# haoheliu/ssr_eval

Measured on AMD Instinct MI355X. Metric: utterance-pairs/sec (LSD+SSIM, 48kHz, n_fft=2048), higher is better.
Workload: dtype f64

## Files before the change

### ssr_eval_amd/csrc/ssr_metrics.h

```cpp
#pragma once
#include "ssr_stft.h"

#define SSR_SSIM_NT 64
#define SSR_SSIM_MAXCPT 6
#define SSR_SSIM_WIN 7

SSR_HD constexpr int ssr_ssim_strip_out(int cpt) { return SSR_SSIM_NT * cpt; }
SSR_HD int ssr_ssim_pick_cpt(int n_bins) {
  const int outs = n_bins - (SSR_SSIM_WIN - 1);
  if (outs <= SSR_SSIM_NT * 4) {
    int c = (outs + SSR_SSIM_NT - 1) / SSR_SSIM_NT;
    return c < 1 ? 1 : c;
  }
  int best = 4, best_waste = 1 << 30;
  for (int c = 4; c <= SSR_SSIM_MAXCPT; ++c) {
    const int w = SSR_SSIM_NT * c;
    const int waste = ((outs + w - 1) / w) * w - outs;
    if (waste < best_waste) { best_waste = waste; best = c; }
  }
  return best;
}

struct SsrSsimParams {
  const float* x;
  const float* y;
  const int64_t* frame_off;
  const int32_t* n_rows;
  int F;
  int rows_per_tile, n_row_tiles, n_strips;
  double* part;
  int pitch;
  int vi_n;
  int64_t x_plane;
};
SSR_DEV int ssr_ssim_pitch(const SsrSsimParams& p) { return p.pitch ? p.pitch : p.F; }

template <int CPT> struct SsrSsimRegs {
  double cs[CPT + 1][4];
  double s;
  float px[2][4][CPT + 1];
  float ring[SSR_SSIM_WIN][CPT + 1];
  double pxy[CPT], pb[CPT];
  float den[CPT];
};

template <int CPT> SSR_DEV int ssr_ssim_slot(int c) { return (CPT % 2 == 0) ? c + c / CPT : c; }
template <int CPT> SSR_DEV int ssr_ssim_slot_of(int tid, int d) { return (CPT % 2 == 0) ? (CPT + 1) * tid + (d + d / CPT) : CPT * tid + d; }

template <int CPT, bool CONTIG = false> struct SsrSsimLds {
  static constexpr int PW = SSR_SSIM_NT * CPT + 8 + ((CPT % 2 == 0) ? (SSR_SSIM_NT * CPT + 8) / CPT + 1 : 0);
  static constexpr int NQ = CONTIG ? 1 : 4;
  static constexpr int RW = SSR_SSIM_NT * CPT + 8;
  static constexpr size_t ring_bytes() { return CONTIG ? sizeof(float) * SSR_SSIM_WIN * RW : 0; }
  static constexpr size_t bytes() { return ring_bytes() + sizeof(double) * (NQ * PW + SSR_SSIM_NT + 16 + 8); }
  float* yring; double* col; double* sc0; double* sc1; double* res;
  SSR_MEMBER explicit SsrSsimLds(char* base) {
    yring = reinterpret_cast<float*>(base);
    col = reinterpret_cast<double*>(base + ring_bytes());
    sc0 = col + NQ * PW;
    sc1 = sc0 + SSR_SSIM_NT;
    res = sc1 + 16;
  }
};

SSR_DEV void ssr_ld4(const float* p, float* o) {
#ifdef SSR_HOST_EMU
  memcpy(o, p, 16);
#else
  typedef float f4 __attribute__((ext_vector_type(4)));
  const f4 v = *reinterpret_cast<const f4*>(p);
  o[0] = v.x; o[1] = v.y; o[2] = v.z; o[3] = v.w;
#endif
}
SSR_DEV void ssr_st4(float* p, const float* v) {
#ifdef SSR_HOST_EMU
  memcpy(p, v, 16);
#else
  typedef float f4 __attribute__((ext_vector_type(4)));
  *reinterpret_cast<f4*>(p) = f4{v[0], v[1], v[2], v[3]};
#endif
}

struct SsrImage {
#ifdef SSR_HOST_EMU
  const float* base;
  SSR_MEMBER SsrImage(const float* p, int64_t) : base(p) {}
// ... 94 lines not shown
    R.cs[i][1] = (R.cs[i][1] + b) - dd;
    R.cs[i][2] = fma(-dd, dd, fma(-c, c, fma(b, b, fma(a, a, R.cs[i][2]))));
    R.cs[i][3] = fma(-c, dd, fma(a, b, R.cs[i][3]));
    R.ring[SLOT][i] = R.px[SET][0][i];
    ssr_touch(R.ring[SLOT][i]);
  }
}

struct SsrSsimK {
  static constexpr double n = 49.0;
  static constexpr float cov = (float)(49.0 / 48.0);
  static constexpr float C1n = (float)((0.01 * 2.0) * (0.01 * 2.0) * 49.0 * 49.0), C2n = (float)((0.03 * 2.0) * (0.03 * 2.0) * 49.0 * 49.0);
};
SSR_DEV void ssr_ssim_stage1(double sx, double sy, double& pxy, double& pp) { pxy = sx * sy; pp = fma(sx, sx, sy * sy); }
SSR_DEV float ssr_ssim_stage2f(double pp, double sq) {
  const double t2 = fma(SsrSsimK::n, sq, -pp);
  const float b1 = (float)pp + SsrSsimK::C1n;
  const float b2 = fmaf(SsrSsimK::cov, (float)t2, SsrSsimK::C2n);
  return b1 * b2;
}
SSR_DEV float ssr_ssim_stage3f(double pxy, double sxy, float b12) {
  const double t1 = fma(SsrSsimK::n, sxy, -pxy);
  const float a1 = fmaf(2.0f, (float)pxy, SsrSsimK::C1n);
  const float a2 = fmaf(2.0f * SsrSsimK::cov, (float)t1, SsrSsimK::C2n);
#ifndef SSR_HOST_EMU
  return (a1 * a2) * __builtin_amdgcn_rcpf(b12);
#else
  return (a1 * a2) / b12;
#endif
}
SSR_DEV double ssr_ssim_value(double sx, double sy, double sq, double sxy) {
  double pxy, pp;
  ssr_ssim_stage1(sx, sy, pxy, pp);
  return (double)ssr_ssim_stage3f(pxy, sxy, ssr_ssim_stage2f(pp, sq));
}

#ifndef SSR_HOST_EMU
#define SSR_SSIM_ST(arr, idx, val) (*(volatile __attribute__((address_space(3))) double*)(&(arr)[idx]) = (val))
#define SSR_SSIM_LD(arr, idx) (*(const volatile __attribute__((address_space(3))) double*)(&(arr)[idx]))
#else
#define SSR_SSIM_ST(arr, idx, val) ((arr)[idx] = (val))
#define SSR_SSIM_LD(arr, idx) ((arr)[idx])
#endif
template <int CPT, bool CONTIG, typename BLK>
SSR_BODY void ssr_ssim_body(const SsrSsimParams& p, BLK& blk, int tile, int item, char* lds_base) {
  constexpr int NT = SSR_SSIM_NT, PW = SsrSsimLds<CPT, CONTIG>::PW, VC = CPT + 1, W = SSR_SSIM_WIN;
  using Regs = SsrSsimRegs<CPT>;
  using Lds = SsrSsimLds<CPT, CONTIG>;
  Lds L(lds_base);
  const int row_tile = tile / p.n_strips, strip = tile % p.n_strips;
  const int item_v = item;
  const float* xbase = p.x;
  if (p.vi_n > 0) { xbase += (int64_t)(item / p.vi_n) * p.x_plane; item = item % p.vi_n; }
  const int T = p.n_rows[item];
  const int out_rows = T - (W - 1);
  const int r0 = row_tile * p.rows_per_tile;
  const int r1 = (r0 + p.rows_per_tile < out_rows) ? r0 + p.rows_per_tile : out_rows;
  const int c_in0 = strip * ssr_ssim_strip_out(CPT);
  const int ncol_in = (p.F - c_in0 < NT * CPT + (W - 1)) ? p.F - c_in0 : NT * CPT + (W - 1);
  const int ncol_out = ncol_in - (W - 1);
  double* part = p.part + (int64_t)item_v * p.n_row_tiles * p.n_strips + tile;
  const int pitch = ssr_ssim_pitch(p);
  const SsrImage x(xbase + p.frame_off[item] * pitch, (int64_t)T * pitch);
  const SsrImage y(p.y + p.frame_off[item] * pitch, (int64_t)T * pitch);

  SSR_REGS(Regs, regs, blk);
  if (r0 >= r1 || ncol_out <= 0) {
    SSR_PHASE(blk, regs, if (tid == 0) *part = 0.0);
    return;
  }
  const int n_steps = (W - 1) + (r1 - r0);
#define SSR_SSIM_STEP(s_, SET, SLOT)                                                                                         \
  SSR_PHASE(blk, regs, {                                                                                                    \
    ssr_ssim_row_apply<CPT, false, SET, SLOT>(R, tid, (s_) >= W, ncol_in);                                                   \
    ssr_ssim_row_load<CPT, false, SET>(p, R, tid, x, y, ssr_ssim_row_ahead(r0 + (s_) + 2, T),                               \
                                       ((s_) + 2 >= W) ? r0 + (s_) + 2 - W : -1, c_in0, ncol_in);                           \
    if ((s_) >= W - 1) {                                                                                                    \
      for (int i = 0; i < VC; ++i) {                                                                                        \
        const int c = ssr_ssim_col<CPT, false>(tid, i);                                                                     \
        if (c < ncol_in)                                                                                                    \
          for (int q = 0; q < 4; ++q) L.col[q * PW + ssr_ssim_slot<CPT>(c)] = R.cs[i][q];                                    \
      }                                                                                                                     \
    }                                                                                                                       \
  });                                                                                                                       \
  if ((s_) >= W - 1) {                                                                                                      \
    SSR_PHASE(blk, regs, {                                                                                                  \
      const int j0 = tid * CPT;                                                                                             \
      if (j0 < ncol_out) {                                                                                                  \
        double w[4][CPT];                                      \
        for (int q = 0; q < 4; ++q) {                                                                                       \
          double v[CPT + W - 1];                                                                                            \
          for (int d = 0; d < CPT + W - 1; ++d) {                                                                           \
            int c = j0 + d;                                                                                                 \
            if (c >= ncol_in) c = ncol_in - 1;                                \
            v[d] = L.col[q * PW + ssr_ssim_slot<CPT>(c)];                                                                   \
          }                                                                                                                 \
          double sw = v[0];                                                                                                 \
          for (int d = 1; d < W; ++d) sw += v[d];                                                                           \
          w[q][0] = sw;                                                                                                     \
          for (int i = 1; i < CPT; ++i) {                                                                                   \
            sw += v[i + W - 1] - v[i - 1];                                                                                  \
            w[q][i] = sw;                                                                                                   \
          }                                                                                                                 \
        }                                                                                                                   \
        for (int i = 0; i < CPT; ++i)                                                                                       \
          if (j0 + i < ncol_out) R.s += ssr_ssim_value(w[0][i], w[1][i], w[2][i], w[3][i]);                                  \
      }                                                                                                                     \
// ... 109 lines not shown
  }
};

template <typename BLK>
SSR_BODY void ssr_specred_body(const SsrSpecRedParams& p, BLK& blk, int chunk, int item, char* lds_base) {
  constexpr int NT = SsrSpecRedLds::NT;
  SsrSpecRedLds L(lds_base);
  const int T = p.n_rows[item];
  const int t0 = chunk * p.rows_per_chunk;
  const int t1 = (t0 + p.rows_per_chunk < T) ? t0 + p.rows_per_chunk : T;
  const float* x = p.x + p.frame_off[item] * p.F;
  const float* y = p.y + p.frame_off[item] * p.F;
  double* part = p.part + ((int64_t)item * p.n_chunks + chunk) * SSR_NPART;
  const bool want_lsd = p.metric_mask & SSR_M_LSD;
  SSR_REGS(SsrSpecRedRegs, regs, blk);
  SSR_PHASE(blk, regs, for (int q = 0; q < 7; ++q) R.acc[q] = 0.0; R.lsd_sum = 0.0);
  for (int t = t0; t < t1; ++t) {
    SSR_PHASE(blk, regs, {
      R.acc[0] = 0.0;
      for (int k = tid; k < p.F; k += NT)
        ssr_accumulate_metrics(x[(int64_t)t * p.F + k], y[(int64_t)t * p.F + k], p.metric_mask, R.acc);
      L.sc0[tid] = R.acc[0];
    });
    if (want_lsd) {
      SSR_PHASE(blk, regs, if (tid < 16) {
        double s = 0.0;
        for (int i = tid; i < NT; i += 16) s += L.sc0[i];
        L.sc1[tid] = s;
      });
      SSR_PHASE(blk, regs, if (tid == 0) {
        double s = 0.0;
        for (int i = 0; i < 16; ++i) s += L.sc1[i];
        R.lsd_sum += sqrt(s / (double)p.F);
      });
    }
  }
#define SSR_GET_ACC(q) R.acc[(q) + 1]
  SSR_BLOCK_SUM(blk, regs, NT, 6, L.sc0, L.sc1, L.res, SSR_GET_ACC);
#undef SSR_GET_ACC
  SSR_PHASE(blk, regs, if (tid == 0) {
    part[0] = R.lsd_sum;
    for (int q = 0; q < 6; ++q) part[1 + q] = L.res[q];
    part[7] = 0.0;
  });
}

struct SsrFinalizeParams {
  const double* part; int n_chunks;
  const double* ssim_part; int n_tiles;
  const int32_t* n_rows;
  int F, metric_mask, n_items;
  double* out;
  int vi_n, out_keys, out_key0;
};

SSR_DEV double ssr_sispec_from_sums(double sdd, double stt, double sdt) {
  const double EPS = 1e-12;
  const double den = stt + EPS;
  const double alpha = (stt + sdt) / den;
  const double beta = (EPS - sdt) / den;
  const double tt = alpha * alpha * stt;
  double nn = sdd + 2.0 * beta * sdt + beta * beta * stt;
  if (nn < 0.0) nn = 0.0;
  return 10.0 * log10(tt / (nn + EPS) + EPS);
}

SSR_DEV void ssr_finalize_item(const SsrFinalizeParams& p, int item) {
  const double nan_ = NAN;
  const int real = p.vi_n > 0 ? item % p.vi_n : item;
  double* o = p.vi_n > 0 ? p.out + ((int64_t)real * p.out_keys + p.out_key0 + item / p.vi_n) * 4 : p.out + (int64_t)item * 4;
  const int T = p.n_rows[real];
  o[0] = o[1] = o[2] = o[3] = nan_;
  if (p.part) {
    double s[SSR_NPART];
    for (int q = 0; q < SSR_NPART; ++q) s[q] = 0.0;
    for (int c = 0; c < p.n_chunks; ++c)
      for (int q = 0; q < SSR_NPART; ++q) s[q] += p.part[((int64_t)item * p.n_chunks + c) * SSR_NPART + q];
    if (p.metric_mask & SSR_M_LSD) o[0] = s[0] / (double)T;
    if (p.metric_mask & SSR_M_LOG_SISPEC) o[1] = ssr_sispec_from_sums(s[4], s[5], s[6]);
    if (p.metric_mask & SSR_M_SISPEC) o[2] = ssr_sispec_from_sums(s[1], s[2], s[3]);
  }
  if (p.ssim_part && (p.metric_mask & SSR_M_SSIM)) {
    double s = 0.0;
    for (int c = 0; c < p.n_tiles; ++c) s += p.ssim_part[(int64_t)item * p.n_tiles + c];
    o[3] = (T >= SSR_SSIM_WIN && p.F >= SSR_SSIM_WIN) ? s / ((double)(T - 6) * (double)(p.F - 6)) : nan_;
  }
}
```

### ssr_eval_amd/csrc/ssr_specred_wave.h

```cpp
#pragma once
#include "ssr_stft.h"

struct SsrSpecWaveParams {
  const float* x;
  const float* y;
  const int64_t* frame_off;
  const int32_t* n_rows;
  int F, pitch, metric_mask, rows_per_chunk, n_chunks, vi_n;
  int64_t x_plane;
  double* part;
};

struct SsrSpecTgt2 { f2 t, tt, lt; };

__device__ __forceinline__ SsrSpecTgt2 ssr_spec_tgt2(float t0, float t1) {
  const f2 t = f2_make(t0, t1);
  return {t, t * t, ssr_log10f_fast2(t + f2_splat(1e-12f))};
}
__device__ __forceinline__ void ssr_spec_tgt_sums2(const SsrSpecTgt2& y, double* tsum) {
  const double t0 = (double)y.t.x, l0 = (double)y.lt.x, t1 = (double)y.t.y, l1 = (double)y.lt.y;
  tsum[0] += t0 * t0; tsum[1] += l0 * l0;
  tsum[0] += t1 * t1; tsum[1] += l1 * l1;
}
__device__ __forceinline__ void ssr_spec_est2(float e0, float e1, const SsrSpecTgt2& y, double* acc) {
  const f2 EPS2 = f2_splat(1e-12f);
  const f2 e = f2_make(e0, e1);
  const f2 ee = e + EPS2;
  const f2 d = ssr_log10f_fast2(ssr_divf_fast2(y.tt, ee * ee) + EPS2);
  const f2 dd = d * d;
  const f2 le = ssr_log10f_fast2(ee);
  {
    acc[0] += (double)dd.x;
    const double td = (double)y.t.x, d0 = (double)e.x - td;
    acc[1] += d0 * d0; acc[3] += d0 * td;
    const double ld = (double)y.lt.x, l0 = (double)le.x - ld;
    acc[4] += l0 * l0; acc[6] += l0 * ld;
  }
  {
    acc[0] += (double)dd.y;
    const double td = (double)y.t.y, d0 = (double)e.y - td;
    acc[1] += d0 * d0; acc[3] += d0 * td;
    const double ld = (double)y.lt.y, l0 = (double)le.y - ld;
    acc[4] += l0 * l0; acc[6] += l0 * ld;
  }
}

template <int KG>
__device__ __forceinline__ void ssr_specred_wave_body(const SsrSpecWaveParams& p, int chunk, int group_v) {
  const int lane = (int)threadIdx.x;
  const int key0 = (group_v / p.vi_n) * KG, item = group_v % p.vi_n;
  const int T = p.n_rows[item];
  const int t0 = chunk * p.rows_per_chunk;
  const int t1 = (t0 + p.rows_per_chunk < T) ? t0 + p.rows_per_chunk : T;
  const float* x = p.x + (int64_t)key0 * p.x_plane + p.frame_off[item] * (int64_t)p.pitch;
  const float* y = p.y + p.frame_off[item] * (int64_t)p.pitch;
  const int mask = p.metric_mask;
  const bool want_lsd = mask & SSR_M_LSD;
  constexpr int FULL = SSR_M_LSD | SSR_M_SISPEC | SSR_M_LOG_SISPEC;
  const bool fast = (mask & FULL) == FULL;
  double acc[KG][7];
  double lsd_sum[KG];
  double tsum[2] = {0.0, 0.0};
#pragma unroll
  for (int g = 0; g < KG; ++g) {
    lsd_sum[g] = 0.0;
#pragma unroll
    for (int q = 0; q < 7; ++q) acc[g][q] = 0.0;
  }
  const int nq = (p.F + 3) / 4;
  const int nfull = p.F / 4;
  for (int t = t0; t < t1; ++t) {
    const float4* yr = reinterpret_cast<const float4*>(y + (int64_t)t * p.pitch);
#pragma unroll
    for (int g = 0; g < KG; ++g) acc[g][0] = 0.0;
    if (fast) {
      for (int q = lane; q < nfull; q += 64) {
        const float4 yv = yr[q];
        float4 xv[KG];
#pragma unroll
        for (int g = 0; g < KG; ++g) xv[g] = reinterpret_cast<const float4*>(x + (int64_t)g * p.x_plane + (int64_t)t * p.pitch)[q];
        const SsrSpecTgt2 y01 = ssr_spec_tgt2(yv.x, yv.y), y23 = ssr_spec_tgt2(yv.z, yv.w);
        ssr_spec_tgt_sums2(y01, tsum);
        ssr_spec_tgt_sums2(y23, tsum);
#pragma unroll
        for (int g = 0; g < KG; ++g) {
          ssr_spec_est2(xv[g].x, xv[g].y, y01, acc[g]);
          ssr_spec_est2(xv[g].z, xv[g].w, y23, acc[g]);
        }
      }
      if (nfull < nq && lane == nfull % 64) {
        const float4 yv = yr[nfull];
        const int k = 4 * nfull;
        double a7[7];
#pragma unroll
        for (int g = 0; g < KG; ++g) {
          const float4 xv = reinterpret_cast<const float4*>(x + (int64_t)g * p.x_plane + (int64_t)t * p.pitch)[nfull];
          a7[0] = acc[g][0]; a7[1] = acc[g][1]; a7[2] = tsum[0]; a7[3] = acc[g][3]; a7[4] = acc[g][4]; a7[5] = tsum[1]; a7[6] = acc[g][6];
          ssr_accumulate_metrics<true>(xv.x, yv.x, mask, a7);
          if (k + 1 < p.F) ssr_accumulate_metrics<true>(xv.y, yv.y, mask, a7);
          if (k + 2 < p.F) ssr_accumulate_metrics<true>(xv.z, yv.z, mask, a7);
          acc[g][0] = a7[0]; acc[g][1] = a7[1]; acc[g][3] = a7[3]; acc[g][4] = a7[4]; acc[g][6] = a7[6];
          if (g == KG - 1) { tsum[0] = a7[2]; tsum[1] = a7[5]; }
        }
      }
// ... 38 lines not shown
```

### ssr_eval_amd/csrc/ssr_stft.h

```cpp
#pragma once
#include "ssr_fft.h"
#define SSR_UIDX(...) ((unsigned)(__VA_ARGS__))

enum { SSR_MODE_PAIR = 0, SSR_MODE_SINGLE = 1 };

SSR_HD constexpr int ssr_stft_ppt(int logn, bool bluestein) { return logn >= 13 ? 16 : 8; }
enum { SSR_OUT_NONE = 0, SSR_OUT_MAG = 1, SSR_OUT_COMPLEX = 2 };
enum { SSR_M_LSD = 1, SSR_M_LOG_SISPEC = 2, SSR_M_SISPEC = 4, SSR_M_SSIM = 8 };

#define SSR_NPART 8

template <typename T> struct SsrStftParams {
  const float* a;
  const double* a64;
  const double* b64;
  const float* b;
  const int64_t* a_off;
  const int64_t* b_off;
  const int32_t* len;
  const int64_t* frame_off;
  int mode, out_kind, metric_mask;
  int n_fft, hop, n_bins;
  int units_per_chunk;
  int n_chunks;
  int interleave;
  const T* window;
  const cx<T>* tw;
  const cx<T>* wchirp;
  const cx<T>* bfilt;
  const cx<T>* chirp;
  float* out_a;
  float* out_b;
  int out_pitch;
  double* part;
};

enum { SSR_IN_F32 = 0, SSR_IN_EST64 = 1, SSR_IN_BOTH64 = 3, SSR_IN_EST64X2 = 7 };
template <bool F64> struct SsrSample { typedef float type; };
template <> struct SsrSample<true> { typedef double type; };

template <typename T, bool SUMS = false, int PPT = 8> struct SsrStftRegs {
  cx<T> v[PPT];
  double sums[SUMS ? 6 : 1];
  cx<T> twp[3 * (PPT >= 8 ? PPT / 8 : 1)];
};

template <typename T, bool SUMS, int PPT, typename SA, typename SB> struct SsrStftRegsPf : SsrStftRegs<T, SUMS, PPT> {
  SA pa[PPT];
  SB pb[PPT];
  T pw[PPT / 2];
};
template <bool BLUESTEIN, typename T, bool SUMS, int PPT, typename SA, typename SB> struct SsrStftPickRegs {
  typedef SsrStftRegsPf<T, SUMS, PPT, SA, SB> type;
};
template <typename T, bool SUMS, int PPT, typename SA, typename SB> struct SsrStftPickRegs<true, T, SUMS, PPT, SA, SB> {
  typedef SsrStftRegs<T, SUMS, PPT> type;
};


SSR_DEV int ssr_num_frames_dev(int n, int n_fft, int hop) { return 1 + (n + 2 * (n_fft / 2) - n_fft) / hop; }

template <typename T> struct SsrBinOut { float ar, ai, br, bi; };

template <typename T> SSR_DEV SsrBinOut<T> ssr_separate(cx<T> zk, cx<T> zn) {
  SsrBinOut<T> o;
  o.ar = (float)(zk.x + zn.x);
  o.ai = (float)(zk.y - zn.y);
  o.br = (float)(zk.y + zn.y);
  o.bi = (float)(zn.x - zk.x);
  return o;
}

SSR_DEV float ssr_cabsf(float re, float im) { return hypotf(re, im); }

SSR_DEV float ssr_cabsf_fast(float re, float im) {
#ifdef SSR_HOST_EMU
  return sqrtf(fmaf(re, re, im * im));
#else
  return __builtin_amdgcn_sqrtf(__builtin_fmaf(re, re, im * im));
#endif
}

SSR_DEV float ssr_divf_fast(float a, float b) {
#ifdef SSR_HOST_EMU
  return a / b;
#else
  const float r = __builtin_amdgcn_rcpf(b);
  const float q = a * r;
  return __builtin_fmaf(__builtin_fmaf(-q, b, a), r, q);
#endif
}
SSR_DEV float ssr_log10f_fast(float x) {
#ifdef SSR_HOST_EMU
  return log10f(x);
#else
  const float y = __builtin_amdgcn_logf(x);
  const float c = 0x1.344134p-2f, cc = 0x1.09f79ep-26f;
  const float r = y * c;
  return r + __builtin_fmaf(y, cc, __builtin_fmaf(y, c, -r));
#endif
}

SSR_DEV f2 ssr_cabsf_fast2(f2 re, f2 im) {
  const f2 s = f2_fma(re, re, im * im);
#ifdef SSR_HOST_EMU
  return f2_make(sqrtf(s.x), sqrtf(s.y));
#else
  return f2_make(__builtin_amdgcn_sqrtf(s.x), __builtin_amdgcn_sqrtf(s.y));
#endif
}
SSR_DEV f2 ssr_divf_fast2(f2 a, f2 b) {
#ifdef SSR_HOST_EMU
  return f2_make(a.x / b.x, a.y / b.y);
// ... 509 lines not shown
```

### ssr_eval_amd/csrc/tu_metrics.hip

```cpp
#include "ssr_host.h"
#include "ssr_metrics.h"
#include "ssr_pair_transform.h"

template <int CPT, bool CONTIG>
__global__ __launch_bounds__(SSR_SSIM_NT, 1) void k_ssim(SsrSsimParams p) {
  extern __shared__ __attribute__((aligned(16))) char smem[];
  SsrBlk blk{(int)threadIdx.x};
  const int tiles = p.n_row_tiles * p.n_strips;
  ssr_ssim_body<CPT, CONTIG>(p, blk, blockIdx.x % tiles, blockIdx.x / tiles, smem);
}


__global__ __launch_bounds__(256) void k_specred(SsrSpecRedParams p) {
  extern __shared__ __attribute__((aligned(16))) char smem[];
  SsrBlk blk{(int)threadIdx.x};
  ssr_specred_body(p, blk, blockIdx.x % p.n_chunks, blockIdx.x / p.n_chunks, smem);
}

__global__ __launch_bounds__(64) void k_finalize(SsrFinalizeParams p) {
  const int item = blockIdx.x * 64 + threadIdx.x;
  if (item < p.n_items) ssr_finalize_item(p, item);
}

struct SsimGeom { int rows_per_tile, n_row_tiles, n_strips, cpt; };
static SsimGeom ssim_geom(int max_rows, int n_bins, int n_items, bool aligned_rows) {
  SsimGeom g;
  const int out_rows = max_rows - 6 > 1 ? max_rows - 6 : 1;
  int64_t r = ((int64_t)out_rows * n_items + ssr_target_wgs() - 1) / ssr_target_wgs();
  if (r < 8) r = 8;
  if (r > 128) r = 128;
  if (r > out_rows) r = out_rows;
  g.rows_per_tile = (int)r;
  g.n_row_tiles = ssr_ceil_div(out_rows, g.rows_per_tile);
  g.cpt = ssr_ssim_pick_cpt(n_bins);
  if (aligned_rows && g.cpt != 4) {
    const int outs = n_bins - (SSR_SSIM_WIN - 1);
    if (outs > 0) {
      const int strips4 = ssr_ceil_div(outs, ssr_ssim_strip_out(4)), strips_c = ssr_ceil_div(outs, ssr_ssim_strip_out(g.cpt));
      if (strips4 * 5 * 68 < strips_c * (g.cpt + 1) * 100) g.cpt = 4;
    }
  }
  g.n_strips = n_bins > 6 ? ssr_ceil_div(n_bins - 6, ssr_ssim_strip_out(g.cpt)) : 1;
  return g;
}


struct PairWs {
  SsrPairGeom g;
  SsimGeom sg;
  SsrPairImages im;
  size_t off_part, off_ssim, total;
};
static PairWs pair_ws(const ssr_plan* pl, int n_items, int max_len, int64_t total_rows, bool in64, bool want_mag) {
  PairWs w;
  w.g = ssr_pair_geom(pl, n_items, max_len, in64);
  w.sg = ssim_geom((int)ssr_num_frames(pl, max_len), pl->n_bins, n_items, true);
  w.im = ssr_pair_images_layout(pl, 1, total_rows, in64, want_mag);
  size_t o = w.im.end;
  w.off_part = o; o += ssr_align256((size_t)n_items * w.g.n_chunks * SSR_NPART * sizeof(double));
  w.off_ssim = o; o += ssr_align256((size_t)n_items * w.sg.n_row_tiles * w.sg.n_strips * sizeof(double));
  w.total = o;
  return w;
}

extern "C" size_t ssr_pair_metrics_workspace_bytes_for(const ssr_plan* pl, int n_items, int max_len, int64_t total_rows,
                                                        unsigned metric_mask) {
  if (!pl || n_items <= 0) return 0;
  const bool mag = metric_mask & SSR_METRIC_SSIM;
  const size_t a = pair_ws(pl, n_items, max_len, total_rows, false, mag).total, b = pair_ws(pl, n_items, max_len, total_rows, true, mag).total;
  return (a > b ? a : b) + ssr_align256((size_t)n_items * sizeof(int32_t));
}

extern "C" size_t ssr_pair_metrics_workspace_bytes(const ssr_plan* pl, int n_items, int max_len, int64_t total_rows) {
  return ssr_pair_metrics_workspace_bytes_for(pl, n_items, max_len, total_rows, SSR_METRIC_ALL);
}

template <int CPT, bool CONTIG = false> static int launch_ssim_inst(const SsrSsimParams& p, int grid, hipStream_t s) {
  const size_t lds = SsrSsimLds<CPT, CONTIG>::bytes();
  static thread_local SsrLdsSlot slot;
  if (int rc = ssr_allow_lds((const void*)k_ssim<CPT, CONTIG>, lds, &slot)) return rc;
  hipLaunchKernelGGL((k_ssim<CPT, CONTIG>), dim3(grid), dim3(SSR_SSIM_NT), lds, s, p);
  HIP_TRY(hipGetLastError());
  return SSR_OK;
}

static int launch_ssim(const float* x, const float* y, const int64_t* frame_off, const int32_t* n_rows, int n_items,
                       int F, int pitch, const SsimGeom& g, double* part, hipStream_t s, int vi_n = 0, int64_t x_plane = 0) {
  SsrSsimParams p{x, y, frame_off, n_rows, F, g.rows_per_tile, g.n_row_tiles, g.n_strips, part, pitch, vi_n, x_plane};
  const int grid = n_items * g.n_row_tiles * g.n_strips;
  if (g.cpt == 4 && pitch > 0 && pitch % 4 == 0 && (((uintptr_t)x | (uintptr_t)y) & 15) == 0)
    return launch_ssim_inst<4, true>(p, grid, s);
  switch (g.cpt) {
    case 1: return launch_ssim_inst<1>(p, grid, s);
    case 2: return launch_ssim_inst<2>(p, grid, s);
    case 3: return launch_ssim_inst<3>(p, grid, s);
    case 4: return launch_ssim_inst<4>(p, grid, s);
    case 5: return launch_ssim_inst<5>(p, grid, s);
    case 6: return launch_ssim_inst<6>(p, grid, s);
  }
  return ssr_fail(SSR_ERR_UNSUPPORTED, "bad SSIM geometry");
}

static int launch_finalize(const double* part, int n_chunks, const double* ssim_part, int n_tiles, const int32_t* n_rows,
                           int F, unsigned mask, int n_items, double* out, hipStream_t s) {
  SsrFinalizeParams p{part, n_chunks, ssim_part, n_tiles, n_rows, F, (int)mask, n_items, out};
  hipLaunchKernelGGL(k_finalize, dim3(ssr_ceil_div(n_items, 64)), dim3(64), 0, s, p);
  HIP_TRY(hipGetLastError());
  return SSR_OK;
}

__global__ void k_rows_from_len(const int32_t* len, int n_items, int n_fft, int hop, int32_t* rows) {
  const int i = blockIdx.x * 256 + threadIdx.x;
  if (i < n_items) rows[i] = ssr_num_frames_dev(len[i], n_fft, hop);
}
int ssr_launch_rows_from_len(const ssr_plan* pl, const int32_t* len, int n_items, int32_t* rows, hipStream_t s) {
  hipLaunchKernelGGL(k_rows_from_len, dim3(ssr_ceil_div(n_items, 256)), dim3(256), 0, s, len, n_items, pl->n_fft, pl->hop, rows);
  HIP_TRY(hipGetLastError());
  return SSR_OK;
}

static int pair_metrics_impl(const ssr_plan* pl, const float* est, const double* est64, const int64_t* est_off,
                             const float* tgt, const double* tgt64, const int64_t* tgt_off, const int32_t* len, const int64_t* frame_off,
                             int n_items, int max_len, int64_t total_rows, unsigned mask, double* out,
                             void* workspace, size_t workspace_bytes, void* stream, int stages) {
  int max_T;
  if (int rc = ssr_check_pair_batch(pl, (est || est64) && (tgt || tgt64) && est_off && tgt_off && len && frame_off && out, n_items, 1, max_len,
                                    mask & SSR_METRIC_SSIM, &max_T))
    return rc;
  if (!max_T) return SSR_OK;
  if ((mask & ~SSR_METRIC_ALL) || mask == 0) return ssr_fail(SSR_ERR_INVALID_ARG, "bad metric mask");
  const bool want_ssim = mask & SSR_METRIC_SSIM;
  if (want_ssim && (max_T < 7 || pl->n_bins < 7)) return ssr_fail(SSR_ERR_INVALID_ARG, "win_size exceeds image extent");
  const PairWs w = pair_ws(pl, n_items, max_len, total_rows, est64 != nullptr, want_ssim);
  const size_t rows_bytes = ssr_align256((size_t)n_items * sizeof(int32_t));
  if (!workspace || workspace_bytes < w.total + rows_bytes) return ssr_fail(SSR_ERR_WORKSPACE, "workspace too small");
  char* ws = (char*)workspace;
  int32_t* rows = (int32_t*)(ws + w.total);
  float *est_plane = (float*)(ws + w.im.off_est), *tgt_plane = (float*)(ws + w.im.off_tgt);
  hipStream_t s = (hipStream_t)stream;
  int rc = SSR_OK;
  if (stages & 1) {
    if ((rc = ssr_launch_rows_from_len(pl, len, n_items, rows, s))) return rc;
    rc = ssr_pair_transform(pl, {len, frame_off, n_items, w.g},
                            {est, est64, est_off, tgt, tgt64, tgt_off, mask, want_ssim ? SSR_OUT_MAG : SSR_OUT_NONE, est_plane, tgt_plane,
                             (double*)(ws + w.off_part)}, s);
    if (rc) return rc;
  }
  if ((stages & 2) && want_ssim) {
    rc = launch_ssim(est_plane, tgt_plane, frame_off, rows, n_items, pl->n_bins, ssr_mag_pitch(pl->n_bins), w.sg, (double*)(ws + w.off_ssim), s);
    if (rc) return rc;
  }
  if (stages & 4) {
    rc = launch_finalize((const double*)(ws + w.off_part), w.g.n_chunks, want_ssim ? (const double*)(ws + w.off_ssim) : nullptr,
                         w.sg.n_row_tiles * w.sg.n_strips, rows, pl->n_bins, mask, n_items, out, s);
  }
  return rc;
}

extern "C" int ssr_pair_metrics_stages(const ssr_plan* pl, const float* est, const int64_t* est_off, const float* tgt,
                                       const int64_t* tgt_off, const int32_t* len, const int64_t* frame_off,
                                       int n_items, int max_len, int64_t total_rows, unsigned mask, double* out,
                                       void* workspace, size_t workspace_bytes, void* stream, int stages) {
  return pair_metrics_impl(pl, est, nullptr, est_off, tgt, nullptr, tgt_off, len, frame_off, n_items, max_len, total_rows,
                           mask, out, workspace, workspace_bytes, stream, stages);
}

extern "C" int ssr_pair_metrics(const ssr_plan* pl, const float* est, const int64_t* est_off, const float* tgt,
                                const int64_t* tgt_off, const int32_t* len, const int64_t* frame_off, int n_items,
                                int max_len, int64_t total_rows, unsigned mask, double* out, void* workspace,
                                size_t workspace_bytes, void* stream) {
  return pair_metrics_impl(pl, est, nullptr, est_off, tgt, nullptr, tgt_off, len, frame_off, n_items, max_len, total_rows,
                           mask, out, workspace, workspace_bytes, stream, 7);
}

extern "C" int ssr_pair_metrics_est64(const ssr_plan* pl, const double* est, const int64_t* est_off, const float* tgt,
                                      const int64_t* tgt_off, const int32_t* len, const int64_t* frame_off, int n_items,
                                      int max_len, int64_t total_rows, unsigned mask, double* out, void* workspace,
                                      size_t workspace_bytes, void* stream) {
  return pair_metrics_impl(pl, nullptr, est, est_off, tgt, nullptr, tgt_off, len, frame_off, n_items, max_len, total_rows,
                           mask, out, workspace, workspace_bytes, stream, 7);
}

extern "C" int ssr_pair_metrics_f64(const ssr_plan* pl, const double* est, const int64_t* est_off, const double* tgt,
                                    const int64_t* tgt_off, const int32_t* len, const int64_t* frame_off, int n_items,
                                    int max_len, int64_t total_rows, unsigned mask, double* out, void* workspace,
                                    size_t workspace_bytes, void* stream) {
  return pair_metrics_impl(pl, nullptr, est, est_off, nullptr, tgt, tgt_off, len, frame_off, n_items, max_len, total_rows,
                           mask, out, workspace, workspace_bytes, stream, 7);
}

#include "ssr_specred_wave.h"
template <int KG> __global__ __launch_bounds__(64) void k_specred_wave(SsrSpecWaveParams p) {
  ssr_specred_wave_body<KG>(p, blockIdx.x % p.n_chunks, blockIdx.x / p.n_chunks);
}

struct MultiWs {
  SsrPairGeom g;
  SsimGeom sg;
  SsrPairImages im;
  size_t off_part_a, off_part_s, off_ssim, off_rows, total;
  int spec_rows_per_chunk, spec_chunks, spec_kg, n_tiles;
  bool fast;
};
static MultiWs multi_ws(const ssr_plan* pl, int n_items, int n_keys, int max_len, int64_t total_rows, unsigned mask, bool est64 = false) {
  MultiWs m;
  const bool want_ssim = mask & SSR_METRIC_SSIM;
  m.fast = ssr_multi_fast_path(pl, est64) && n_keys > 1;
  m.g = ssr_pair_geom(pl, n_items, max_len, est64);
  const int max_T = (int)ssr_num_frames(pl, max_len);
  m.sg = ssim_geom(max_T, pl->n_bins, m.fast ? n_items * n_keys : n_items, true);
  m.n_tiles = m.sg.n_row_tiles * m.sg.n_strips;
  m.im = ssr_pair_images_layout(pl, n_keys, total_rows, est64, want_ssim || m.fast, false);
  const int n_spec = ((n_keys - 1) / 2) * 2;
  m.spec_kg = ssr_keys_per_wave(n_spec);
  m.spec_rows_per_chunk = ssr_wave_rows_per_wg(max_T, (int64_t)n_items * (n_spec > 0 ? n_spec / m.spec_kg : 1));
  m.spec_chunks = ssr_ceil_div(max_T, m.spec_rows_per_chunk);
  size_t o = m.im.end;
  m.off_part_a = o; o += 2 * ssr_align256((size_t)n_items * m.g.n_chunks * SSR_NPART * sizeof(double));
  m.off_part_s = o; o += ssr_align256((size_t)n_items * n_keys * m.spec_chunks * SSR_NPART * sizeof(double));
  m.off_ssim = o; o += ssr_align256((size_t)n_items * n_keys * m.n_tiles * sizeof(double));
  m.off_rows = o; o += ssr_align256((size_t)n_items * sizeof(int32_t));
  m.total = o;
  return m;
}

extern "C" size_t ssr_pair_metrics_multi_workspace_bytes(const ssr_plan* pl, int n_items, int n_keys, int max_len, int64_t total_rows,
                                                         unsigned metric_mask) {
  if (!pl || n_items <= 0 || n_keys <= 0) return 0;
  return multi_ws(pl, n_items, n_keys, max_len, total_rows, metric_mask).total;
}

static int pair_metrics_multi_impl(const ssr_plan* pl, const float* est, const double* est64, const int64_t* est_off, const float* tgt,
                                   const int64_t* tgt_off, const int32_t* len, const int64_t* frame_off, int n_items, int n_keys, int max_len,
                                   int64_t total_rows, unsigned mask, double* out, void* workspace, size_t workspace_bytes, void* stream) {
  int max_T;
  if (int rc = ssr_check_pair_batch(pl, (est || est64) && est_off && tgt && tgt_off && len && frame_off && out, n_items, n_keys, max_len, true,
                                    &max_T))
    return rc;
  if (!max_T) return SSR_OK;
  if ((mask & ~SSR_METRIC_ALL) || mask == 0) return ssr_fail(SSR_ERR_INVALID_ARG, "bad metric mask");
  const bool want_ssim = mask & SSR_METRIC_SSIM;
  if (want_ssim && (max_T < 7 || pl->n_bins < 7)) return ssr_fail(SSR_ERR_INVALID_ARG, "win_size exceeds image extent");
  const MultiWs m = multi_ws(pl, n_items, n_keys, max_len, total_rows, mask, est64 != nullptr);
  if (!workspace || workspace_bytes < m.total) return ssr_fail(SSR_ERR_WORKSPACE, "workspace too small");
  char* ws = (char*)workspace;
  hipStream_t s = (hipStream_t)stream;
  int32_t* rows = (int32_t*)(ws + m.off_rows);
  int rc;
  if ((rc = ssr_launch_rows_from_len(pl, len, n_items, rows, s))) return rc;
  const SsrPairBatch bt{len, frame_off, n_items, m.g};
  const bool mag = m.im.plane != 0;
  const int pitch = ssr_mag_pitch(pl->n_bins);
  const int64_t plane_floats = (int64_t)(m.im.plane / sizeof(float));
  const unsigned red_mask = mask & (SSR_METRIC_LSD | SSR_METRIC_LOG_SISPEC | SSR_METRIC_SISPEC);
  auto plane_of = [&](int k) { return mag ? (float*)(ws + m.im.off_est + (size_t)k * m.im.plane) : nullptr; };
  float* tgt_plane = mag ? (float*)(ws + m.im.off_tgt) : nullptr;
  double* part0 = (double*)(ws + m.off_part_a);
  double* ssim_part = (double*)(ws + m.off_ssim);
  auto finalize = [&](const double* part, int n_chunks, const double* sp, int n_virtual, int key0) {
    SsrFinalizeParams p{part, n_chunks, want_ssim ? sp : nullptr, m.n_tiles, rows, pl->n_bins, (int)mask, n_virtual, out, n_items, n_keys, key0};
    hipLaunchKernelGGL(k_finalize, dim3(ssr_ceil_div(n_virtual, 64)), dim3(64), 0, s, p);
    return hipGetLastError();
  };
  auto ssim = [&](int key0, int n_k) {
    return launch_ssim(plane_of(key0), tgt_plane, frame_off, rows, n_items * n_k, pl->n_bins, pitch, m.sg,
                       ssim_part + (size_t)key0 * n_items * m.n_tiles, s, n_items, plane_floats);
  };
  if (!m.fast) {
    for (int k = 0; k < n_keys; ++k) {
      rc = ssr_pair_transform(pl, bt, {est, est64, est_off + (size_t)k * n_items, tgt, nullptr, tgt_off, mask, mag ? SSR_OUT_MAG : SSR_OUT_NONE,
                                       plane_of(k), tgt_plane, part0}, s);
      if (rc) return rc;
      if (want_ssim && (rc = ssim(k, 1))) return rc;
      HIP_TRY(finalize(part0, m.g.n_chunks, ssim_part + (size_t)k * n_items * m.n_tiles, n_items, k));
    }
    return SSR_OK;
  }
  const int n_spec = ((n_keys - 1) / 2) * 2;
  const int k_last = n_spec + 1;
  const bool odd_last = k_last < n_keys;
  double* part_last = (double*)(ws + m.off_part_a + ssr_align256((size_t)n_items * m.g.n_chunks * SSR_NPART * sizeof(double)));
  if ((rc = ssr_pair_images(pl, bt, est, est64, est_off, tgt, tgt_off, n_keys, m.im, ws, s, mask, part0, part_last))) return rc;
  if (n_spec > 0 && red_mask) {
    SsrSpecWaveParams q{plane_of(1), tgt_plane, frame_off, rows, pl->n_bins, pitch, (int)red_mask, m.spec_rows_per_chunk, m.spec_chunks, n_items,
                        plane_floats, (double*)(ws + m.off_part_s)};
    const int kg = m.spec_kg;
    const dim3 grid((unsigned)((int64_t)(n_spec / kg) * n_items * m.spec_chunks));
    if (kg == 3) hipLaunchKernelGGL(k_specred_wave<3>, grid, dim3(64), 0, s, q);
    else if (kg == 2) hipLaunchKernelGGL(k_specred_wave<2>, grid, dim3(64), 0, s, q);
    else hipLaunchKernelGGL(k_specred_wave<1>, grid, dim3(64), 0, s, q);
    HIP_TRY(hipGetLastError());
  }
  if (want_ssim && (rc = ssim(0, n_keys))) return rc;
  HIP_TRY(finalize(part0, m.g.n_chunks, ssim_part, n_items, 0));
  if (n_spec > 0)
    HIP_TRY(finalize(red_mask ? (const double*)(ws + m.off_part_s) : nullptr, m.spec_chunks, ssim_part + (size_t)n_items * m.n_tiles, n_spec * n_items, 1));
  if (odd_last) HIP_TRY(finalize(part_last, m.g.n_chunks, ssim_part + (size_t)k_last * n_items * m.n_tiles, n_items, k_last));
  return SSR_OK;
}

extern "C" int ssr_pair_metrics_multi(const ssr_plan* pl, const float* est, const int64_t* est_off, const float* tgt, const int64_t* tgt_off,
                                      const int32_t* len, const int64_t* frame_off, int n_items, int n_keys, int max_len, int64_t total_rows,
                                      unsigned mask, double* out, void* workspace, size_t workspace_bytes, void* stream) {
  if (!est) return ssr_fail(SSR_ERR_INVALID_ARG, "null argument");
  return pair_metrics_multi_impl(pl, est, nullptr, est_off, tgt, tgt_off, len, frame_off, n_items, n_keys, max_len, total_rows, mask, out,
                                 workspace, workspace_bytes, stream);
}

extern "C" size_t ssr_pair_metrics_multi_est64_workspace_bytes(const ssr_plan* pl, int n_items, int n_keys, int max_len, int64_t total_rows,
                                                               unsigned metric_mask) {
  if (!pl || n_items <= 0 || n_keys <= 0) return 0;
  return multi_ws(pl, n_items, n_keys, max_len, total_rows, metric_mask, true).total;
}
extern "C" int ssr_pair_metrics_multi_est64(const ssr_plan* pl, const double* est, const int64_t* est_off, const float* tgt, const int64_t* tgt_off,
                                            const int32_t* len, const int64_t* frame_off, int n_items, int n_keys, int max_len,
                                            int64_t total_rows, unsigned mask, double* out, void* workspace, size_t workspace_bytes,
                                            void* stream) {
  if (!est) return ssr_fail(SSR_ERR_INVALID_ARG, "null argument");
  return pair_metrics_multi_impl(pl, nullptr, est, est_off, tgt, tgt_off, len, frame_off, n_items, n_keys, max_len, total_rows, mask, out,
                                 workspace, workspace_bytes, stream);
}

struct SpecWs { size_t off_part, off_ssim, total; int rows_per_chunk, n_chunks; SsimGeom sg; };
static SpecWs spec_ws(int n_items, int max_rows, int n_bins) {
  SpecWs w;
  w.rows_per_chunk = ssr_units_per_chunk_for(max_rows, n_items);
  w.n_chunks = ssr_ceil_div(max_rows, w.rows_per_chunk);
  w.sg = ssim_geom(max_rows, n_bins, n_items, false);
  size_t o = 0;
  w.off_part = o; o += ssr_align256((size_t)n_items * w.n_chunks * SSR_NPART * sizeof(double));
  w.off_ssim = o; o += ssr_align256((size_t)n_items * w.sg.n_row_tiles * w.sg.n_strips * sizeof(double));
  w.total = o;
  return w;
}

extern "C" size_t ssr_spectrogram_metrics_workspace_bytes(int n_items, int max_rows, int n_bins) {
  if (n_items <= 0) return 0;
  return spec_ws(n_items, max_rows, n_bins).total;
}

extern "C" int ssr_spectrogram_metrics(const float* est_sp, const float* tgt_sp, const int64_t* frame_off,
                                       const int32_t* n_rows, int n_items, int max_rows, int n_bins, unsigned mask,
                                       double* out, void* workspace, size_t workspace_bytes, void* stream) {
  if (!est_sp || !tgt_sp || !frame_off || !n_rows || !out) return ssr_fail(SSR_ERR_INVALID_ARG, "null argument");
  if (n_items <= 0) return SSR_OK;
  if ((mask & ~SSR_METRIC_ALL) || mask == 0) return ssr_fail(SSR_ERR_INVALID_ARG, "bad metric mask");
  if (max_rows < 1 || n_bins < 1) return ssr_fail(SSR_ERR_INVALID_ARG, "empty spectrogram");
  if ((int64_t)max_rows * n_bins >= ((int64_t)1 << 30))
    return ssr_fail(SSR_ERR_UNSUPPORTED, "spectrogram of 2^30 elements or more (4 GiB buffer views)");
  const bool want_ssim = mask & SSR_METRIC_SSIM;
  if (want_ssim && (max_rows < 7 || n_bins < 7)) return ssr_fail(SSR_ERR_INVALID_ARG, "win_size exceeds image extent");
  const SpecWs w = spec_ws(n_items, max_rows, n_bins);
  if (!workspace || workspace_bytes < w.total) return ssr_fail(SSR_ERR_WORKSPACE, "workspace too small");
  char* ws = (char*)workspace;
  hipStream_t s = (hipStream_t)stream;
  const bool want_red = mask & (SSR_METRIC_LSD | SSR_METRIC_SISPEC | SSR_METRIC_LOG_SISPEC);
  if (want_red) {
    SsrSpecRedParams p{est_sp, tgt_sp, frame_off, n_rows, n_bins, (int)mask, w.rows_per_chunk, w.n_chunks,
                       (double*)(ws + w.off_part)};
    hipLaunchKernelGGL(k_specred, dim3(n_items * w.n_chunks), dim3(256), SsrSpecRedLds::bytes(), s, p);
    HIP_TRY(hipGetLastError());
  }
  if (want_ssim) {
    int rc = launch_ssim(est_sp, tgt_sp, frame_off, n_rows, n_items, n_bins, 0, w.sg, (double*)(ws + w.off_ssim), s);
    if (rc) return rc;
  }
  return launch_finalize(want_red ? (const double*)(ws + w.off_part) : nullptr, w.n_chunks,
                         want_ssim ? (const double*)(ws + w.off_ssim) : nullptr, w.sg.n_row_tiles * w.sg.n_strips, n_rows,
                         n_bins, mask, n_items, out, s);
}
```

Measured before the change: 343,400.

## Pick SSIM row tiles by occupancy wave cost and compute frame counts inline

Adds an occupancy-aware SSIM tiling picker. For non-ragged batches it searches rows-per-tile to minimise the count of resident-wave rounds times the tile height plus halo, using the HIP occupancy query and CU count, with results cached per device. It also drops the separate rows-from-length kernel launch and the workspace buffer it wrote: kernels now derive frame counts from the lengths on the fly. This saves one launch per call and should give better wave balance, at the cost of a small amount of extra device arithmetic and a host occupancy query on first use.

```diff
diff --git a/ssr_eval_amd/csrc/ssr_metrics.h b/ssr_eval_amd/csrc/ssr_metrics.h
--- a/ssr_eval_amd/csrc/ssr_metrics.h
+++ b/ssr_eval_amd/csrc/ssr_metrics.h
@@ -32,6 +32,8 @@
   int pitch;
   int vi_n;
   int64_t x_plane;
+  const int32_t* len;
+  int n_fft, hop;
 };
 SSR_DEV int ssr_ssim_pitch(const SsrSsimParams& p) { return p.pitch ? p.pitch : p.F; }
 
@@ -232,7 +234,7 @@
   const int item_v = item;
   const float* xbase = p.x;
   if (p.vi_n > 0) { xbase += (int64_t)(item / p.vi_n) * p.x_plane; item = item % p.vi_n; }
-  const int T = p.n_rows[item];
+  const int T = ssr_item_rows(p.n_rows, p.len, p.n_fft, p.hop, item);
   const int out_rows = T - (W - 1);
   const int r0 = row_tile * p.rows_per_tile;
   const int r1 = (r0 + p.rows_per_tile < out_rows) ? r0 + p.rows_per_tile : out_rows;
@@ -448,6 +450,8 @@
   int F, metric_mask, n_items;
   double* out;
   int vi_n, out_keys, out_key0;
+  const int32_t* len;
+  int n_fft, hop;
 };
 
 SSR_DEV double ssr_sispec_from_sums(double sdd, double stt, double sdt) {
@@ -465,7 +469,7 @@
   const double nan_ = NAN;
   const int real = p.vi_n > 0 ? item % p.vi_n : item;
   double* o = p.vi_n > 0 ? p.out + ((int64_t)real * p.out_keys + p.out_key0 + item / p.vi_n) * 4 : p.out + (int64_t)item * 4;
-  const int T = p.n_rows[real];
+  const int T = ssr_item_rows(p.n_rows, p.len, p.n_fft, p.hop, real);
   o[0] = o[1] = o[2] = o[3] = nan_;
   if (p.part) {
     double s[SSR_NPART];
diff --git a/ssr_eval_amd/csrc/ssr_specred_wave.h b/ssr_eval_amd/csrc/ssr_specred_wave.h
--- a/ssr_eval_amd/csrc/ssr_specred_wave.h
+++ b/ssr_eval_amd/csrc/ssr_specred_wave.h
@@ -9,6 +9,8 @@
   int F, pitch, metric_mask, rows_per_chunk, n_chunks, vi_n;
   int64_t x_plane;
   double* part;
+  const int32_t* len;
+  int n_fft, hop;
 };
 
 struct SsrSpecTgt2 { f2 t, tt, lt; };
@@ -49,7 +51,7 @@
 __device__ __forceinline__ void ssr_specred_wave_body(const SsrSpecWaveParams& p, int chunk, int group_v) {
   const int lane = (int)threadIdx.x;
   const int key0 = (group_v / p.vi_n) * KG, item = group_v % p.vi_n;
-  const int T = p.n_rows[item];
+  const int T = ssr_item_rows(p.n_rows, p.len, p.n_fft, p.hop, item);
   const int t0 = chunk * p.rows_per_chunk;
   const int t1 = (t0 + p.rows_per_chunk < T) ? t0 + p.rows_per_chunk : T;
   const float* x = p.x + (int64_t)key0 * p.x_plane + p.frame_off[item] * (int64_t)p.pitch;
diff --git a/ssr_eval_amd/csrc/ssr_ssim_geom.h b/ssr_eval_amd/csrc/ssr_ssim_geom.h
--- /dev/null
+++ b/ssr_eval_amd/csrc/ssr_ssim_geom.h
@@ -0,0 +1,44 @@
+#pragma once
+#include <cstdint>
+
+#define SSR_SSIM_GEOM_LANES 64
+#define SSR_SSIM_GEOM_HALO 6
+#define SSR_SSIM_GEOM_MIN_ROWS 8
+#define SSR_SSIM_GEOM_MAX_ROWS 128
+#define SSR_SSIM_GEOM_TARGET_WGS 4096
+
+struct SsrSsimTiles { int rows_per_tile, n_row_tiles, n_strips; };
+
+inline int ssr_ssim_geom_out_rows(int rows) { return rows - SSR_SSIM_GEOM_HALO > 1 ? rows - SSR_SSIM_GEOM_HALO : 1; }
+
+inline int ssr_ssim_geom_fixed_rows(int out_rows, int n_items) {
+  int64_t r = ((int64_t)out_rows * n_items + SSR_SSIM_GEOM_TARGET_WGS - 1) / SSR_SSIM_GEOM_TARGET_WGS;
+  if (r < SSR_SSIM_GEOM_MIN_ROWS) r = SSR_SSIM_GEOM_MIN_ROWS;
+  if (r > SSR_SSIM_GEOM_MAX_ROWS) r = SSR_SSIM_GEOM_MAX_ROWS;
+  if (r > out_rows) r = out_rows;
+  return (int)r;
+}
+
+inline SsrSsimTiles ssr_ssim_geom_pick(int max_rows, int mean_rows, int n_items, int n_bins, int cpt, int64_t resident_waves) {
+  SsrSsimTiles g;
+  const int out_rows = ssr_ssim_geom_out_rows(max_rows);
+  const int strip_out = SSR_SSIM_GEOM_LANES * (cpt > 0 ? cpt : 1);
+  g.n_strips = n_bins > SSR_SSIM_GEOM_HALO ? (n_bins - SSR_SSIM_GEOM_HALO + strip_out - 1) / strip_out : 1;
+  g.rows_per_tile = ssr_ssim_geom_fixed_rows(out_rows, n_items);
+  const bool ragged = (int64_t)max_rows * 10 > (int64_t)mean_rows * 11;
+  if (!ragged && resident_waves > 0 && out_rows >= SSR_SSIM_GEOM_MIN_ROWS && n_items > 0) {
+    const int mean_out = ssr_ssim_geom_out_rows(mean_rows);
+    int64_t best_cost = -1;
+    for (int nt = 1; nt <= out_rows; ++nt) {
+      const int r = (out_rows + nt - 1) / nt;
+      if (r > SSR_SSIM_GEOM_MAX_ROWS) continue;
+      if (r < SSR_SSIM_GEOM_MIN_ROWS) break;
+      if ((out_rows + r - 1) / r != nt) continue;
+      const int64_t waves = (int64_t)n_items * g.n_strips * ((mean_out + r - 1) / r);
+      const int64_t cost = ((waves + resident_waves - 1) / resident_waves) * (r + SSR_SSIM_GEOM_HALO);
+      if (best_cost < 0 || cost < best_cost) { best_cost = cost; g.rows_per_tile = r; }
+    }
+  }
+  g.n_row_tiles = (out_rows + g.rows_per_tile - 1) / g.rows_per_tile;
+  return g;
+}
diff --git a/ssr_eval_amd/csrc/ssr_stft.h b/ssr_eval_amd/csrc/ssr_stft.h
--- a/ssr_eval_amd/csrc/ssr_stft.h
+++ b/ssr_eval_amd/csrc/ssr_stft.h
@@ -59,6 +59,9 @@
 
 
 SSR_DEV int ssr_num_frames_dev(int n, int n_fft, int hop) { return 1 + (n + 2 * (n_fft / 2) - n_fft) / hop; }
+SSR_DEV int ssr_item_rows(const int32_t* n_rows, const int32_t* len, int n_fft, int hop, int i) {
+  return n_rows ? n_rows[i] : ssr_num_frames_dev(len[i], n_fft, hop);
+}
 
 template <typename T> struct SsrBinOut { float ar, ai, br, bi; };
 
diff --git a/ssr_eval_amd/csrc/tu_metrics.hip b/ssr_eval_amd/csrc/tu_metrics.hip
--- a/ssr_eval_amd/csrc/tu_metrics.hip
+++ b/ssr_eval_amd/csrc/tu_metrics.hip
@@ -1,6 +1,9 @@
 #include "ssr_host.h"
 #include "ssr_metrics.h"
 #include "ssr_pair_transform.h"
+#include "ssr_ssim_geom.h"
+
+#include <atomic>
 
 template <int CPT, bool CONTIG>
 __global__ __launch_bounds__(SSR_SSIM_NT, 1) void k_ssim(SsrSsimParams p) {
@@ -23,15 +26,46 @@
 }
 
 struct SsimGeom { int rows_per_tile, n_row_tiles, n_strips, cpt; };
-static SsimGeom ssim_geom(int max_rows, int n_bins, int n_items, bool aligned_rows) {
+static_assert(SSR_SSIM_GEOM_LANES == SSR_SSIM_NT && SSR_SSIM_GEOM_HALO == SSR_SSIM_WIN - 1, "ssr_ssim_geom.h restates the kernel's strip");
+
+template <int CPT, bool CONTIG> static int ssim_blocks_per_cu() {
+  int nb = 0;
+  if (hipOccupancyMaxActiveBlocksPerMultiprocessor(&nb, k_ssim<CPT, CONTIG>, SSR_SSIM_NT, SsrSsimLds<CPT, CONTIG>::bytes()) != hipSuccess) {
+    (void)hipGetLastError();
+    return 0;
+  }
+  return nb;
+}
+static int64_t ssim_resident_waves(int device, int cpt, bool contig) {
+  enum { MAX_DEV = 32, N_INST = SSR_SSIM_MAXCPT + 2 };
+  static std::atomic<int64_t> cache[MAX_DEV][N_INST];
+  const int inst = contig ? 0 : cpt;
+  const bool tracked = device >= 0 && device < MAX_DEV && inst >= 0 && inst < N_INST;
+  if (tracked) {
+    const int64_t c = cache[device][inst].load(std::memory_order_relaxed);
+    if (c != 0) return c > 0 ? c : 0;
+  }
+  int nb = 0, cus = 0;
+  if (contig) nb = ssim_blocks_per_cu<4, true>();
+  else switch (cpt) {
+    case 1: nb = ssim_blocks_per_cu<1, false>(); break;
+    case 2: nb = ssim_blocks_per_cu<2, false>(); break;
+    case 3: nb = ssim_blocks_per_cu<3, false>(); break;
+    case 4: nb = ssim_blocks_per_cu<4, false>(); break;
+    case 5: nb = ssim_blocks_per_cu<5, false>(); break;
+    case 6: nb = ssim_blocks_per_cu<6, false>(); break;
+  }
+  if (nb > 0 && hipDeviceGetAttribute(&cus, hipDeviceAttributeMultiprocessorCount, device) != hipSuccess) {
+    (void)hipGetLastError();
+    cus = 0;
+  }
+  const int64_t w = nb > 0 && cus > 0 ? (int64_t)nb * cus : -1;
+  if (tracked) cache[device][inst].store(w, std::memory_order_relaxed);
+  return w > 0 ? w : 0;
+}
+
+static SsimGeom ssim_geom(int device, int max_rows, int mean_rows, int n_bins, int n_items, bool aligned_rows) {
   SsimGeom g;
-  const int out_rows = max_rows - 6 > 1 ? max_rows - 6 : 1;
-  int64_t r = ((int64_t)out_rows * n_items + ssr_target_wgs() - 1) / ssr_target_wgs();
-  if (r < 8) r = 8;
-  if (r > 128) r = 128;
-  if (r > out_rows) r = out_rows;
-  g.rows_per_tile = (int)r;
-  g.n_row_tiles = ssr_ceil_div(out_rows, g.rows_per_tile);
   g.cpt = ssr_ssim_pick_cpt(n_bins);
   if (aligned_rows && g.cpt != 4) {
     const int outs = n_bins - (SSR_SSIM_WIN - 1);
@@ -40,9 +74,14 @@
       if (strips4 * 5 * 68 < strips_c * (g.cpt + 1) * 100) g.cpt = 4;
     }
   }
-  g.n_strips = n_bins > 6 ? ssr_ceil_div(n_bins - 6, ssr_ssim_strip_out(g.cpt)) : 1;
+  const int64_t resident = device >= 0 ? ssim_resident_waves(device, g.cpt, aligned_rows && g.cpt == 4) : 0;
+  const SsrSsimTiles t = ssr_ssim_geom_pick(max_rows, mean_rows, n_items, n_bins, g.cpt, resident);
+  g.rows_per_tile = t.rows_per_tile;
+  g.n_row_tiles = t.n_row_tiles;
+  g.n_strips = t.n_strips;
   return g;
 }
+static int ssim_mean_rows(int64_t total_rows, int n_items) { return n_items > 0 && total_rows > 0 ? (int)(total_rows / n_items) : 0; }
 
 
 struct PairWs {
@@ -54,7 +93,7 @@
 static PairWs pair_ws(const ssr_plan* pl, int n_items, int max_len, int64_t total_rows, bool in64, bool want_mag) {
   PairWs w;
   w.g = ssr_pair_geom(pl, n_items, max_len, in64);
-  w.sg = ssim_geom((int)ssr_num_frames(pl, max_len), pl->n_bins, n_items, true);
+  w.sg = ssim_geom(pl->device, (int)ssr_num_frames(pl, max_len), ssim_mean_rows(total_rows, n_items), pl->n_bins, n_items, true);
   w.im = ssr_pair_images_layout(pl, 1, total_rows, in64, want_mag);
   size_t o = w.im.end;
   w.off_part = o; o += ssr_align256((size_t)n_items * w.g.n_chunks * SSR_NPART * sizeof(double));
@@ -68,7 +107,7 @@
   if (!pl || n_items <= 0) return 0;
   const bool mag = metric_mask & SSR_METRIC_SSIM;
   const size_t a = pair_ws(pl, n_items, max_len, total_rows, false, mag).total, b = pair_ws(pl, n_items, max_len, total_rows, true, mag).total;
-  return (a > b ? a : b) + ssr_align256((size_t)n_items * sizeof(int32_t));
+  return a > b ? a : b;
 }
 
 extern "C" size_t ssr_pair_metrics_workspace_bytes(const ssr_plan* pl, int n_items, int max_len, int64_t total_rows) {
@@ -84,9 +123,12 @@
   return SSR_OK;
 }
 
-static int launch_ssim(const float* x, const float* y, const int64_t* frame_off, const int32_t* n_rows, int n_items,
+struct RowsSrc { const int32_t* n_rows; const int32_t* len; int n_fft, hop; };
+static RowsSrc rows_of_len(const ssr_plan* pl, const int32_t* len) { return {nullptr, len, pl->n_fft, pl->hop}; }
+static int launch_ssim(const float* x, const float* y, const int64_t* frame_off, const RowsSrc& rows, int n_items,
                        int F, int pitch, const SsimGeom& g, double* part, hipStream_t s, int vi_n = 0, int64_t x_plane = 0) {
-  SsrSsimParams p{x, y, frame_off, n_rows, F, g.rows_per_tile, g.n_row_tiles, g.n_strips, part, pitch, vi_n, x_plane};
+  SsrSsimParams p{x, y, frame_off, rows.n_rows, F, g.rows_per_tile, g.n_row_tiles, g.n_strips, part, pitch, vi_n, x_plane,
+                  rows.len, rows.n_fft, rows.hop};
   const int grid = n_items * g.n_row_tiles * g.n_strips;
   if (g.cpt == 4 && pitch > 0 && pitch % 4 == 0 && (((uintptr_t)x | (uintptr_t)y) & 15) == 0)
     return launch_ssim_inst<4, true>(p, grid, s);
@@ -101,9 +143,9 @@
   return ssr_fail(SSR_ERR_UNSUPPORTED, "bad SSIM geometry");
 }
 
-static int launch_finalize(const double* part, int n_chunks, const double* ssim_part, int n_tiles, const int32_t* n_rows,
+static int launch_finalize(const double* part, int n_chunks, const double* ssim_part, int n_tiles, const RowsSrc& rows,
                            int F, unsigned mask, int n_items, double* out, hipStream_t s) {
-  SsrFinalizeParams p{part, n_chunks, ssim_part, n_tiles, n_rows, F, (int)mask, n_items, out};
+  SsrFinalizeParams p{part, n_chunks, ssim_part, n_tiles, rows.n_rows, F, (int)mask, n_items, out, 0, 0, 0, rows.len, rows.n_fft, rows.hop};
   hipLaunchKernelGGL(k_finalize, dim3(ssr_ceil_div(n_items, 64)), dim3(64), 0, s, p);
   HIP_TRY(hipGetLastError());
   return SSR_OK;
@@ -132,15 +174,13 @@
   const bool want_ssim = mask & SSR_METRIC_SSIM;
   if (want_ssim && (max_T < 7 || pl->n_bins < 7)) return ssr_fail(SSR_ERR_INVALID_ARG, "win_size exceeds image extent");
   const PairWs w = pair_ws(pl, n_items, max_len, total_rows, est64 != nullptr, want_ssim);
-  const size_t rows_bytes = ssr_align256((size_t)n_items * sizeof(int32_t));
-  if (!workspace || workspace_bytes < w.total + rows_bytes) return ssr_fail(SSR_ERR_WORKSPACE, "workspace too small");
+  if (!workspace || workspace_bytes < w.total) return ssr_fail(SSR_ERR_WORKSPACE, "workspace too small");
   char* ws = (char*)workspace;
-  int32_t* rows = (int32_t*)(ws + w.total);
+  const RowsSrc rows = rows_of_len(pl, len);
   float *est_plane = (float*)(ws + w.im.off_est), *tgt_plane = (float*)(ws + w.im.off_tgt);
   hipStream_t s = (hipStream_t)stream;
   int rc = SSR_OK;
   if (stages & 1) {
-    if ((rc = ssr_launch_rows_from_len(pl, len, n_items, rows, s))) return rc;
     rc = ssr_pair_transform(pl, {len, frame_off, n_items, w.g},
                             {est, est64, est_off, tgt, tgt64, tgt_off, mask, want_ssim ? SSR_OUT_MAG : SSR_OUT_NONE, est_plane, tgt_plane,
                              (double*)(ws + w.off_part)}, s);
@@ -198,7 +238,7 @@
   SsrPairGeom g;
   SsimGeom sg;
   SsrPairImages im;
-  size_t off_part_a, off_part_s, off_ssim, off_rows, total;
+  size_t off_part_a, off_part_s, off_ssim, total;
   int spec_rows_per_chunk, spec_chunks, spec_kg, n_tiles;
   bool fast;
 };
@@ -208,7 +248,7 @@
   m.fast = ssr_multi_fast_path(pl, est64) && n_keys > 1;
   m.g = ssr_pair_geom(pl, n_items, max_len, est64);
   const int max_T = (int)ssr_num_frames(pl, max_len);
-  m.sg = ssim_geom(max_T, pl->n_bins, m.fast ? n_items * n_keys : n_items, true);
+  m.sg = ssim_geom(pl->device, max_T, ssim_mean_rows(total_rows, n_items), pl->n_bins, m.fast ? n_items * n_keys : n_items, true);
   m.n_tiles = m.sg.n_row_tiles * m.sg.n_strips;
   m.im = ssr_pair_images_layout(pl, n_keys, total_rows, est64, want_ssim || m.fast, false);
   const int n_spec = ((n_keys - 1) / 2) * 2;
@@ -219,7 +259,6 @@
   m.off_part_a = o; o += 2 * ssr_align256((size_t)n_items * m.g.n_chunks * SSR_NPART * sizeof(double));
   m.off_part_s = o; o += ssr_align256((size_t)n_items * n_keys * m.spec_chunks * SSR_NPART * sizeof(double));
   m.off_ssim = o; o += ssr_align256((size_t)n_items * n_keys * m.n_tiles * sizeof(double));
-  m.off_rows = o; o += ssr_align256((size_t)n_items * sizeof(int32_t));
   m.total = o;
   return m;
 }
@@ -245,9 +284,8 @@
   if (!workspace || workspace_bytes < m.total) return ssr_fail(SSR_ERR_WORKSPACE, "workspace too small");
   char* ws = (char*)workspace;
   hipStream_t s = (hipStream_t)stream;
-  int32_t* rows = (int32_t*)(ws + m.off_rows);
+  const RowsSrc rows = rows_of_len(pl, len);
   int rc;
-  if ((rc = ssr_launch_rows_from_len(pl, len, n_items, rows, s))) return rc;
   const SsrPairBatch bt{len, frame_off, n_items, m.g};
   const bool mag = m.im.plane != 0;
   const int pitch = ssr_mag_pitch(pl->n_bins);
@@ -258,7 +296,8 @@
   double* part0 = (double*)(ws + m.off_part_a);
   double* ssim_part = (double*)(ws + m.off_ssim);
   auto finalize = [&](const double* part, int n_chunks, const double* sp, int n_virtual, int key0) {
-    SsrFinalizeParams p{part, n_chunks, want_ssim ? sp : nullptr, m.n_tiles, rows, pl->n_bins, (int)mask, n_virtual, out, n_items, n_keys, key0};
+    SsrFinalizeParams p{part, n_chunks, want_ssim ? sp : nullptr, m.n_tiles, nullptr, pl->n_bins, (int)mask, n_virtual, out, n_items, n_keys, key0,
+                        len, pl->n_fft, pl->hop};
     hipLaunchKernelGGL(k_finalize, dim3(ssr_ceil_div(n_virtual, 64)), dim3(64), 0, s, p);
     return hipGetLastError();
   };
@@ -282,8 +321,8 @@
   double* part_last = (double*)(ws + m.off_part_a + ssr_align256((size_t)n_items * m.g.n_chunks * SSR_NPART * sizeof(double)));
   if ((rc = ssr_pair_images(pl, bt, est, est64, est_off, tgt, tgt_off, n_keys, m.im, ws, s, mask, part0, part_last))) return rc;
   if (n_spec > 0 && red_mask) {
-    SsrSpecWaveParams q{plane_of(1), tgt_plane, frame_off, rows, pl->n_bins, pitch, (int)red_mask, m.spec_rows_per_chunk, m.spec_chunks, n_items,
-                        plane_floats, (double*)(ws + m.off_part_s)};
+    SsrSpecWaveParams q{plane_of(1), tgt_plane, frame_off, nullptr, pl->n_bins, pitch, (int)red_mask, m.spec_rows_per_chunk, m.spec_chunks, n_items,
+                        plane_floats, (double*)(ws + m.off_part_s), len, pl->n_fft, pl->hop};
     const int kg = m.spec_kg;
     const dim3 grid((unsigned)((int64_t)(n_spec / kg) * n_items * m.spec_chunks));
     if (kg == 3) hipLaunchKernelGGL(k_specred_wave<3>, grid, dim3(64), 0, s, q);
@@ -326,7 +365,7 @@
   SpecWs w;
   w.rows_per_chunk = ssr_units_per_chunk_for(max_rows, n_items);
   w.n_chunks = ssr_ceil_div(max_rows, w.rows_per_chunk);
-  w.sg = ssim_geom(max_rows, n_bins, n_items, false);
+  w.sg = ssim_geom(-1, max_rows, 0, n_bins, n_items, false);
   size_t o = 0;
   w.off_part = o; o += ssr_align256((size_t)n_items * w.n_chunks * SSR_NPART * sizeof(double));
   w.off_ssim = o; o += ssr_align256((size_t)n_items * w.sg.n_row_tiles * w.sg.n_strips * sizeof(double));
@@ -362,10 +401,10 @@
     HIP_TRY(hipGetLastError());
   }
   if (want_ssim) {
-    int rc = launch_ssim(est_sp, tgt_sp, frame_off, n_rows, n_items, n_bins, 0, w.sg, (double*)(ws + w.off_ssim), s);
+    int rc = launch_ssim(est_sp, tgt_sp, frame_off, RowsSrc{n_rows, nullptr, 0, 0}, n_items, n_bins, 0, w.sg, (double*)(ws + w.off_ssim), s);
     if (rc) return rc;
   }
   return launch_finalize(want_red ? (const double*)(ws + w.off_part) : nullptr, w.n_chunks,
-                         want_ssim ? (const double*)(ws + w.off_ssim) : nullptr, w.sg.n_row_tiles * w.sg.n_strips, n_rows,
-                         n_bins, mask, n_items, out, s);
-}
+                         want_ssim ? (const double*)(ws + w.off_ssim) : nullptr, w.sg.n_row_tiles * w.sg.n_strips,
+                         RowsSrc{n_rows, nullptr, 0, 0}, n_bins, mask, n_items, out, s);
+}
```

New measurement: 344,500 (median of 4 runs). No clear change (+0.3%).
